# Chang-Tun-Yu/HLS-final-Visual-Odometry

Hardware: AMD Instinct MI355X
Metric: stereo frame-pairs/sec (detect+match), KITTI 1241x376; matches bit-exact (higher is better)
Workload: dtype u8; 1 GPU; KITTI 1241x376 stereo quad-match (prev/curr x L/R), default 50x50 bins; noise=0, gpu_max_hw_queues=4, streams_per_gpu=256, frames_in_hbm=8, parallelism=1x independent stream groups

## Files before the change

hls-final-visual-odometry_amd/csrc/kernels_match.hip:

```cpp
#include "vh_findmatch.h"
#include <algorithm>
#include <cstdlib>
#include <type_traits>

#ifdef VH_FLOW_STATS
__device__ unsigned long long g_flow_stats[12];
extern "C" int32_t vh_debug_flow_stats(unsigned long long *out, int32_t reset) {
  if (hipMemcpyFromSymbol(out, HIP_SYMBOL(g_flow_stats), sizeof(g_flow_stats)) != hipSuccess) return -3;
  if (reset) { unsigned long long z[12] = {0}; if (hipMemcpyToSymbol(HIP_SYMBOL(g_flow_stats), z, sizeof(z)) != hipSuccess) return -3; }
  return 0;
}
#define VH_STAT(k, n) do { if ((threadIdx.x & 63) == 0) atomicAdd(&g_flow_stats[k], (unsigned long long)(n)); } while (0)
#else
#define VH_STAT(k, n) do { } while (0)
#endif

#ifndef VH_MATCH_WAVES
#define VH_MATCH_WAVES 7
#endif
#ifndef VH_SNAKE
#define VH_SNAKE 1
#endif

namespace {

__device__ __forceinline__ int32_t wave_min(int32_t v) {
#pragma unroll
  for (int32_t d = 32; d >= 1; d >>= 1) v = min(v, __shfl_xor(v, d));
  return v;
}
__device__ __forceinline__ int32_t wave_max(int32_t v) {
#pragma unroll
  for (int32_t d = 32; d >= 1; d >>= 1) v = max(v, __shfl_xor(v, d));
  return v;
}

template <bool MAX>
__device__ __forceinline__ int32_t row16_allreduce(int32_t v) {
#define VH_ROW_STEP(CTRL)                                                                   \
  {                                                                                         \
    const int32_t t = __builtin_amdgcn_update_dpp(v, v, CTRL, 0xF, 0xF, false);             \
    v = MAX ? max(v, t) : min(v, t);                                                        \
  }
  VH_ROW_STEP(0x128)
  VH_ROW_STEP(0x124)
  VH_ROW_STEP(0x122)
  VH_ROW_STEP(0x121)
#undef VH_ROW_STEP
  return v;
}

template <class T>
__device__ __forceinline__ T ld_off(const T *base, uint32_t byte_off) { return *(const T *)((const char *)base + byte_off); }
template <class T>
__device__ __forceinline__ void st_off(T *base, uint32_t byte_off, T x) { *(T *)((char *)base + byte_off) = x; }
template <class T>
__device__ __forceinline__ T ld_uniform(const T *p) { return *(const __attribute__((address_space(4))) T *)(uintptr_t)p; }
__device__ __forceinline__ int32_t ld_uniform_i32(const int32_t *p) { return __builtin_amdgcn_readfirstlane(ld_uniform(p)); }

template <bool TESTED, class First, class Step>
__device__ __forceinline__ void walk_columns(const VhSets &s, const int32_t *__restrict__ cbs, int32_t c, int32_t UB0, int32_t UB1, int32_t VB0,
                                             int32_t VB1, int32_t ULO_MAX, int32_t UHI_MIN, int32_t VA0, int32_t VA1, First first, Step step) {
  const int32_t lane = threadIdx.x & 63;
  const bool merged = !TESTED && VB0 == 0 && VB1 == s.vbn - 1;
  const int32_t UB1w = merged ? UB0 : UB1;
  for (int32_t cb = UB0; cb <= UB1w; cb += 64) {
    const int32_t ncb = min(64, UB1w - cb + 1);
    int32_t t_p0 = 0, t_p1 = 0, t_a0 = 0, t_a1 = 0;
    if (lane < ncb) {
      const int32_t row = (c * s.ubn + cb + lane) * s.vbn;
      t_p0 = ld_off(cbs, (uint32_t)(row + VB0) * 4u);
      t_p1 = ld_off(cbs, (uint32_t)(merged ? (c * s.ubn + UB1 + 1) * s.vbn : row + VB1 + 1) * 4u);
      if (TESTED) {
        const int32_t ubx = cb + lane;
        const bool in_ = ubx * s.binsize >= ULO_MAX && ubx * s.binsize + s.binsize - 1 <= UHI_MIN;
        t_a0 = in_ ? ((VA0 <= VA1) ? cbs[row + VA0] : t_p1) : 1;
        t_a1 = in_ ? ((VA0 <= VA1) ? cbs[row + VA1 + 1] : t_p1) : 0;
      }
    }
    int32_t ci = -1, pc = -64, p1 = 0;
    const auto advance = [&]() -> bool {
      pc += 64;
      while (pc >= p1) {
        if (++ci >= ncb) return false;
        pc = __builtin_amdgcn_readlane(t_p0, ci); p1 = __builtin_amdgcn_readlane(t_p1, ci);
      }
      return true;
    };
    if (!advance()) continue;
    first(pc, p1);
    for (;;) {
      const int32_t c_pc = pc, c_p1 = p1, c_ci = ci;
      const bool more = advance();
      int32_t pa0 = 1, pa1 = 0;
      if (TESTED) { pa0 = __builtin_amdgcn_readlane(t_a0, c_ci); pa1 = __builtin_amdgcn_readlane(t_a1, c_ci); }
      step(c_pc, c_p1, pa0, pa1, more, pc, p1);
      if (!more) break;
    }
  }
}

template <bool TESTED, bool NEED_UV, class Consume>
__device__ __forceinline__ void walk_region(const VhSets &s, const int32_t *__restrict__ cbs, const uint32_t *__restrict__ cuv,
                                            const uint4 *__restrict__ cdesc, int32_t c, int32_t UB0, int32_t UB1, int32_t VB0,
                                            int32_t VB1, int32_t ULO_MAX, int32_t UHI_MIN, int32_t VA0, int32_t VA1,
                                            Consume consume) {
  const int32_t lane = threadIdx.x & 63;
  int32_t pl = 0;
  uint32_t gu = 0;
  uint4 g0, g1;
  const auto load = [&](int32_t pc, int32_t p1) __attribute__((always_inline)) {
    pl = min(pc + lane, p1 - 1);
    if (NEED_UV) gu = cuv[pl];
    g0 = cdesc[2 * (int64_t)pl]; g1 = cdesc[2 * (int64_t)pl + 1];
  };
  walk_columns<TESTED>(s, cbs, c, UB0, UB1, VB0, VB1, ULO_MAX, UHI_MIN, VA0, VA1, load,
    [&](int32_t pc, int32_t p1, int32_t pa0, int32_t pa1, bool more, int32_t npc, int32_t np1) __attribute__((always_inline)) {
      const int32_t c_pl = pl;
      const uint32_t c_gu = gu;
      const uint4 c_g0 = g0, c_g1 = g1;
      if (more) load(npc, np1);
      consume(pc, p1, pa0, pa1, c_pl, c_gu, c_g0, c_g1);
    });
}

__device__ __forceinline__ void glds16(const void *gbase, uint32_t byte_off, uint32_t lds_dst) {
  asm volatile("s_mov_b32 m0, %2\n\ts_nop 0\n\tglobal_load_lds_dwordx4 %0, %1" ::"v"(byte_off), "s"(gbase), "s"(lds_dst) : "memory");
}
__device__ __forceinline__ void glds4(const void *gbase, uint32_t byte_off, uint32_t lds_dst) {
  asm volatile("s_mov_b32 m0, %2\n\ts_nop 0\n\tglobal_load_lds_dword %0, %1" ::"v"(byte_off), "s"(gbase), "s"(lds_dst) : "memory");
}
__device__ __forceinline__ uint32_t lds_addr(const void *p) {
  return __builtin_amdgcn_readfirstlane((uint32_t)(uintptr_t)(const __attribute__((address_space(3))) void *)p);
}

template <bool TESTED, class Consume>
__device__ __forceinline__ void walk_region_lds(const VhSets &s, const int32_t *__restrict__ cbs, const uint32_t *__restrict__ cuv,
                                                const uint4 *__restrict__ cdesc, int32_t c, int32_t UB0, int32_t UB1, int32_t VB0,
                                                int32_t VB1, int32_t ULO_MAX, int32_t UHI_MIN, int32_t VA0, int32_t VA1,
                                                uint4 *wD, uint32_t *wU, Consume consume) {
  const uint32_t ldsD = lds_addr(wD), ldsU = lds_addr(wU);
  const uint32_t lane32 = (uint32_t)(threadIdx.x & 63) * 32u;
  const auto issue = [&](int32_t b, int32_t pc, int32_t p1) __attribute__((always_inline)) {
    const uint32_t off = min((uint32_t)pc * 32u + lane32, (uint32_t)(p1 - 1) * 32u);
    glds16(cdesc, off, ldsD + (uint32_t)b * 2048u); glds16(cdesc, off + 16u, ldsD + (uint32_t)b * 2048u + 1024u);
    if (TESTED) glds4(cuv, off >> 3, ldsU + (uint32_t)b * 256u);
  };
  int32_t buf = 0;
  walk_columns<TESTED>(s, cbs, c, UB0, UB1, VB0, VB1, ULO_MAX, UHI_MIN, VA0, VA1,
    [&](int32_t pc, int32_t p1) __attribute__((always_inline)) {
      asm volatile("s_waitcnt lgkmcnt(0)" ::: "memory");
      buf = 0;
      issue(0, pc, p1);
    },
    [&](int32_t pc, int32_t p1, int32_t pa0, int32_t pa1, bool more, int32_t npc, int32_t np1) __attribute__((always_inline)) {
      const int32_t c_buf = buf;
      if (more) {
        buf ^= 1;
        asm volatile("s_waitcnt lgkmcnt(0)" ::: "memory");
        issue(buf, npc, np1);
        if (TESTED) asm volatile("s_waitcnt vmcnt(3)" ::: "memory");
        else asm volatile("s_waitcnt vmcnt(2)" ::: "memory");
      } else {
        asm volatile("s_waitcnt vmcnt(0)" ::: "memory");
      }
      consume(pc, p1, pa0, pa1, (const uint4 *)(wD + c_buf * 128), (const uint32_t *)(wU + c_buf * 64));
    });
}

__device__ __forceinline__ uint64_t tested_key_uniform_query(const uint32_t (&qd)[8], us2 lo2, us2 span2, uint32_t uv2,
                                                             const uint4 &b0, const uint4 &b1, uint32_t relpos) {
  const bool out = outside_window(uv2, lo2, span2);
  const uint32_t sad = sad32(make_uint4(qd[0], qd[1], qd[2], qd[3]), make_uint4(qd[4], qd[5], qd[6], qd[7]), b0, b1, 0);
  return out ? ~0ull : (((uint64_t)sad << 32) | relpos);
}
__device__ __forceinline__ uint64_t shfl_xor_u64(uint64_t k, int32_t d) {
  const uint32_t lo = (uint32_t)__shfl_xor((int32_t)(uint32_t)k, d), hi = (uint32_t)__shfl_xor((int32_t)(uint32_t)(k >> 32), d);
  return ((uint64_t)hi << 32) | lo;
}
__device__ __forceinline__ uint64_t wave_min_u64(uint64_t k) {
#pragma unroll
  for (int32_t d = 32; d >= 1; d >>= 1) k = min(k, shfl_xor_u64(k, d));
  return k;
}

enum { KEY_HI16 = 0, KEY_W19 = 1, KEY_64 = 2 };
template <int KM> struct KeyT { typedef uint32_t type; };
template <> struct KeyT<KEY_64> { typedef uint64_t type; };
template <int KM>
__device__ __forceinline__ typename KeyT<KM>::type sad_key(const uint4 &a0, const uint4 &a1, const uint4 &b0, const uint4 &b1, uint32_t seed) {
  if (KM == KEY_HI16) return (typename KeyT<KM>::type)sad32<true>(a0, a1, b0, b1, seed);
  const uint32_t sad = sad32(a0, a1, b0, b1, 0);
  if (KM == KEY_W19) return (typename KeyT<KM>::type)((sad << 19) | seed);
  return (typename KeyT<KM>::type)(((uint64_t)sad << 32) | seed);
}
__device__ __forceinline__ int32_t key_mode_of(int32_t class_count, int32_t wide_keys) {
  if (class_count + 64 <= 0x10000 && !wide_keys) return KEY_HI16;
  return class_count <= VH_CLASS_POS_MAX && wide_keys < 2 ? KEY_W19 : KEY_64;
}

template <int Q, int P, int KM>
__device__ __forceinline__ int32_t join_phases(const typename KeyT<KM>::type (&best_key)[Q]) {
  static_assert(Q == 2 && P == 4, "the join splits the wave into two slots of two 16-lane rows");
  if (KM == KEY_64) {
    uint64_t k[Q];
#pragma unroll
    for (int32_t qi = 0; qi < Q; qi++) {
      k[qi] = (uint64_t)best_key[qi];
#pragma unroll
      for (int32_t d = 16; d < 64; d <<= 1) k[qi] = min(k[qi], shfl_xor_u64(k[qi], d));
    }
    const uint64_t kk = (threadIdx.x & 32) ? k[1] : k[0];
    return kk == ~0ull ? -1 : (int32_t)(uint32_t)kk;
  }
  const auto h = __builtin_amdgcn_permlane32_swap((uint32_t)best_key[0], (uint32_t)best_key[1], false, false);
  const uint32_t kh = min(h[0], h[1]);
  const auto r = __builtin_amdgcn_permlane16_swap(kh, kh, false, false);
  const uint32_t k = min(r[0], r[1]);
  return k == 0xFFFFFFFFu ? -1 : (int32_t)(k & (KM == KEY_HI16 ? 0xFFFFu : 0x7FFFFu));
}

#ifndef VH_REDO_G
#define VH_REDO_G 2
#endif
struct RedoGroup {
  uint32_t qd[VH_REDO_G][8];
  us2 lo2[VH_REDO_G];
  int32_t lane[VH_REDO_G], n;
  int32_t umin, umax, vmin, vmax;
};
template <int Q>
__device__ __forceinline__ bool redo_take(uint64_t &todo, const uint4 (&a0)[Q], const uint4 (&a1)[Q], const uint32_t (&uv1)[Q],
                                          int32_t radius, int32_t rv, RedoGroup &g) {
  g.n = 0; g.umin = g.vmin = 0x7FFFFFFF; g.umax = g.vmax = -1;
#pragma unroll
  for (int32_t k = 0; k < VH_REDO_G; k++) {
    if (!todo) break;
    const int32_t fl = (int32_t)__builtin_ctzll(todo), fq = fl >> 5;
    todo &= todo - 1;
    uint4 x0 = a0[0], x1 = a1[0];
    uint32_t xu = uv1[0];
#pragma unroll
    for (int32_t qi = 1; qi < Q; qi++) if (fq == qi) { x0 = a0[qi]; x1 = a1[qi]; xu = uv1[qi]; }
    g.qd[k][0] = __builtin_amdgcn_readlane(x0.x, fl); g.qd[k][1] = __builtin_amdgcn_readlane(x0.y, fl);
    g.qd[k][2] = __builtin_amdgcn_readlane(x0.z, fl); g.qd[k][3] = __builtin_amdgcn_readlane(x0.w, fl);
    g.qd[k][4] = __builtin_amdgcn_readlane(x1.x, fl); g.qd[k][5] = __builtin_amdgcn_readlane(x1.y, fl);
    g.qd[k][6] = __builtin_amdgcn_readlane(x1.z, fl); g.qd[k][7] = __builtin_amdgcn_readlane(x1.w, fl);
    const uint32_t quv1 = __builtin_amdgcn_readlane(xu, fl);
    const int32_t u1 = (int32_t)(quv1 & 0xFFFF), v1 = (int32_t)(quv1 >> 16);
    g.lo2[k] = window_lo2(quv1, radius, rv);
    g.lane[k] = fl; g.n = k + 1;
    g.umin = min(g.umin, u1); g.umax = max(g.umax, u1); g.vmin = min(g.vmin, v1); g.vmax = max(g.vmax, v1);
  }
  return g.n > 0;
}

template <int Q> struct TileOut {
  int32_t wp;
  uint4 a0[Q], a1[Q];
  uint32_t uv1[Q];
  int32_t qpos[Q];
  bool valid[Q];
};

template <int Q, int P, bool SPEC, bool FLOW>
__device__ __forceinline__ void finish_tile(const VhSets &s, const VhMatchArgs &a, int32_t pass, int32_t stream, int32_t qset, int32_t cset,
                                            int32_t c, int32_t pbase, int32_t pcnt, const TileOut<Q> &o,
                                            int32_t *__restrict__ best, int32_t *__restrict__ redo_count) {
  static_assert(Q == 2 && P == 4, "one query per lane: slot lane >> 5, on the first 16-lane row of each half (join_phases)");
  const int32_t lane = threadIdx.x & 63;
  const uint32_t *__restrict__ cuv = s.s_uv + (int64_t)cset * s.cap;
  const uint4 *__restrict__ cdesc = (const uint4 *)(s.s_desc + (int64_t)cset * s.cap * 8);
  const int32_t *__restrict__ cbs = s.bin_start + (int64_t)cset * (s.nbins + 1);
  const int32_t rv = FLOW ? a.radius : a.disp_tol;
  const us2 span2 = window_span2(a.radius, rv);
  const int32_t *__restrict__ cidx = s.s_idx + (int64_t)cset * s.cap;
  const int32_t *__restrict__ qidx = s.s_idx + (int64_t)qset * s.cap;
  int32_t *__restrict__ tbl = best + ((int64_t)stream * 4 + a.pass[pass].slot) * s.cap;
  const bool hi = lane & 32;
  const bool mine = !(lane & 16) && (hi ? o.valid[1] : o.valid[0]);
  const uint32_t uv1 = hi ? o.uv1[1] : o.uv1[0];
  const int32_t qpos = hi ? o.qpos[1] : o.qpos[0];
  int32_t res = -1;
  bool fail = false;
  if (mine && o.wp >= 0) {
    int32_t wp = o.wp;
    VH_CHECK_RANGE(s, 7, wp, 0, pcnt);
    res = pbase + wp;
    if (SPEC) fail = outside_window(ld_off(cuv, (uint32_t)res * 4u), window_lo2(uv1, a.radius, rv), span2);
  }
  if (SPEC) {
    uint64_t todo = __ballot(fail);
    if (todo) {
      const int32_t nfail = (int32_t)__popcll(todo);
      VH_STAT(FLOW ? 7 : 10, nfail);
      if (lane == 0) atomicAdd(redo_count, nfail);
      RedoGroup g;
      while (redo_take<Q>(todo, o.a0, o.a1, o.uv1, a.radius, rv, g)) {
        uint64_t kk[VH_REDO_G];
#pragma unroll
        for (int32_t k = 0; k < VH_REDO_G; k++) kk[k] = ~0ull;
        if (FLOW) {
          const VhBins b = bins_of_interest(s, VhWindow{g.umin - a.radius, g.umax + a.radius, g.vmin - rv, g.vmax + rv});
          walk_region<false, true>(s, cbs, cuv, cdesc, c, b.ub0, b.ub1, b.vb0, b.vb1, 0, 0, 0, 0,
            [&](int32_t, int32_t, int32_t, int32_t, int32_t pl, uint32_t gu, const uint4 &g0, const uint4 &g1) {
#pragma unroll
              for (int32_t k = 0; k < VH_REDO_G; k++)
                if (k < g.n) kk[k] = min(kk[k], tested_key_uniform_query(g.qd[k], g.lo2[k], span2, gu, g0, g1, (uint32_t)(pl - pbase)));
            });
        } else {
          const int32_t *__restrict__ crs = s.row_start + (int64_t)cset * (4 * s.H + 1);
          const int32_t *__restrict__ cpos = s.r_pos + (int64_t)cset * s.cap;
          const int32_t x0 = ld_uniform_i32(crs + c * s.H + max(g.vmin - rv, 0));
          const int32_t x1 = ld_uniform_i32(crs + c * s.H + min(g.vmax + rv, s.H - 1) + 1);
          for (int32_t x = x0 + lane; x < x1; x += 64) {
            int32_t cp = cpos[x];
            VH_CHECK_RANGE(s, 3, cp, pbase, pbase + pcnt);
            const uint32_t gu = cuv[cp];
            const uint4 g0 = cdesc[2 * (int64_t)cp], g1 = cdesc[2 * (int64_t)cp + 1];
#pragma unroll
            for (int32_t k = 0; k < VH_REDO_G; k++)
              if (k < g.n) kk[k] = min(kk[k], tested_key_uniform_query(g.qd[k], g.lo2[k], span2, gu, g0, g1, (uint32_t)(cp - pbase)));
          }
        }
#pragma unroll
        for (int32_t k = 0; k < VH_REDO_G; k++)
          if (k < g.n) {
            const uint64_t kf = wave_min_u64(kk[k]);
            int32_t wp = (int32_t)(uint32_t)kf;
            if (kf != ~0ull) VH_CHECK_RANGE(s, 7, wp, 0, pcnt);
            if (lane == g.lane[k]) res = kf == ~0ull ? -1 : pbase + wp;
          }
      }
    }
  }
  if (mine) st_off(tbl, (uint32_t)ld_off(qidx, (uint32_t)qpos * 4u) * 4u, res < 0 ? 0 : ld_off(cidx, (uint32_t)res * 4u));
}

template <int Q, int P, int KM, bool SPEC>
__device__ __forceinline__ void flow_tile(const VhSets &s, const VhMatchArgs &a, int32_t pass, int32_t stream,
                                          int32_t qset, int32_t cset, int32_t q0, int32_t q1, int32_t c, int32_t col0,
                                          int32_t pbase, int32_t pcnt, uint4 *wD, uint32_t *wU, TileOut<Q> &out) {
  constexpr int L = 64 / P;
  static_assert(L == 8 || L == 16, "every 16-lane row must hold the whole tile (row-wise window reduction)");
  constexpr int TRIP = 2 * P;
  const int32_t lane = threadIdx.x & 63, ph = lane / L, l = lane % L;
  const uint32_t *__restrict__ quv = s.s_uv + (int64_t)qset * s.cap;
  const uint4 *__restrict__ qdesc = (const uint4 *)(s.s_desc + (int64_t)qset * s.cap * 8);
  const uint32_t *__restrict__ cuv = s.s_uv + (int64_t)cset * s.cap;
  const uint4 *__restrict__ cdesc = (const uint4 *)(s.s_desc + (int64_t)cset * s.cap * 8);
  const int32_t *__restrict__ cbs = s.bin_start + (int64_t)cset * (s.nbins + 1);
  const int32_t rv = a.pass[pass].flow ? a.radius : a.disp_tol;

  bool (&valid)[Q] = out.valid;
  uint4 (&a0)[Q] = out.a0, (&a1)[Q] = out.a1;
  uint32_t (&uv1)[Q] = out.uv1;
  int32_t v_lo[Q];
  us2 lo2[Q];
  typedef typename KeyT<KM>::type key_t;
  const key_t KNONE = (key_t)~(key_t)0;
  key_t best_key[Q];
  int32_t umin = 0x7FFFFFFF, umax = -1, vmin = 0x7FFFFFFF, vmax = -1;
  int32_t (&qp)[Q] = out.qpos;
#pragma unroll
  for (int32_t qi = 0; qi < Q; qi++) {
    const int32_t q = q0 + L * qi + l;
    valid[qi] = q < q1;
    qp[qi] = valid[qi] ? q : q0;
  }
  {
    const int32_t *__restrict__ qbs = s.bin_start + (int64_t)qset * (s.nbins + 1);
    int32_t colb = col0, j = 0;
    int32_t csv = ld_off(qbs, (uint32_t)((c * s.ubn + min(colb + lane, s.ubn)) * s.vbn) * 4u);
    int32_t A = __builtin_amdgcn_readlane(csv, 0);
    int32_t k[Q];
#pragma unroll
    for (int32_t qi = 0; qi < Q; qi++) k[qi] = qp[qi];
    for (;;) {
      const int32_t B = __builtin_amdgcn_readlane(csv, j + 1);
      if (VH_SNAKE && ((colb + j) & 1)) {
#pragma unroll
        for (int32_t qi = 0; qi < Q; qi++) if (k[qi] >= A && k[qi] < B) qp[qi] = A + B - 1 - k[qi];
      }
      if (B >= q1 || colb + j + 1 >= s.ubn) break;
      A = B;
      if (++j == 63) { colb += 63; j = 0; csv = ld_off(qbs, (uint32_t)((c * s.ubn + min(colb + lane, s.ubn)) * s.vbn) * 4u); }
    }
  }
#pragma unroll
  for (int32_t qi = 0; qi < Q; qi++) {
    const int32_t ql = qp[qi];
    uv1[qi] = ld_off(quv, (uint32_t)ql * 4u);
    a0[qi] = ld_off(qdesc, (uint32_t)ql * 32u); a1[qi] = ld_off(qdesc, (uint32_t)ql * 32u + 16u);
    const int32_t u1 = uv1[qi] & 0xFFFF, v1 = uv1[qi] >> 16;
    v_lo[qi] = v1 - rv;
    lo2[qi] = window_lo2(uv1[qi], a.radius, rv);
    best_key[qi] = KNONE;
    umin = min(umin, u1); umax = max(umax, u1); vmin = min(vmin, v1); vmax = max(vmax, v1);
  }
  umin = __builtin_amdgcn_readfirstlane(row16_allreduce<false>(umin));
  umax = __builtin_amdgcn_readfirstlane(row16_allreduce<true>(umax));
  vmin = __builtin_amdgcn_readfirstlane(row16_allreduce<false>(vmin));
  vmax = __builtin_amdgcn_readfirstlane(row16_allreduce<true>(vmax));
  const VhBins ub = bins_of_interest(s, VhWindow{umin - a.radius, umax + a.radius, vmin - rv, vmax + rv});
  const int32_t UB0 = ub.ub0, UB1 = ub.ub1, VB0 = ub.vb0, VB1 = ub.vb1;
  const us2 span2 = window_span2(a.radius, rv);
  const int32_t ULO_MAX = umax - a.radius, UHI_MIN = umin + a.radius;
  const int32_t VLO_MAX = vmax - rv, VHI_MIN = vmin + rv;
  const int32_t VA0 = SPEC ? 0 : max(VB0, (max(VLO_MAX, 0) + s.binsize - 1) / s.binsize);
  const int32_t VA1 = SPEC ? 0 : min(VB1, (VHI_MIN + 1) / s.binsize - 1);

  auto make_key = [&](auto test, int32_t qi, uint32_t uv2, const uint4 &b0, const uint4 &b1, uint32_t seed) -> key_t {
    constexpr int TEST = decltype(test)::value;
    bool out = false;
    if (TEST == 2) {
      out = outside_window(uv2, lo2[qi], span2);
    } else if (TEST == 1) {
      out = (uint32_t)((int32_t)(uv2 >> 16) - v_lo[qi]) > (uint32_t)(2 * rv);
    }
    const key_t key = sad_key<KM>(a0[qi], a1[qi], b0, b1, seed);
    return (TEST != 0 && out) ? KNONE : key;
  };
  VH_STAT(0, 1); VH_STAT(5, q1 - q0); VH_STAT(6, UB1 - UB0 + 1);
  walk_region_lds<!SPEC>(s, cbs, cuv, cdesc, c, UB0, UB1, VB0, VB1, ULO_MAX, UHI_MIN, VA0, VA1, wD, wU,
    [&](int32_t pc, int32_t p1, int32_t pa0, int32_t pa1, const uint4 *cD, const uint32_t *cU) {
      VH_STAT(1, 1);
      const int32_t mcnt = min(64, p1 - pc);
      const int32_t jend = (mcnt + TRIP - 1) & ~(TRIP - 1);
      const uint4 *rd = cD + ph;
      const uint32_t *ru = cU + ph;
      uint32_t seedA = (uint32_t)(pc - pbase + ph), seedB = seedA + P;
      int32_t j = 0;
      auto trip = [&](auto test, int32_t o) {
        const uint4 dA0 = rd[o], dA1 = rd[o + 64], dB0 = rd[o + P], dB1 = rd[o + 64 + P];
        uint32_t uA = 0, uB = 0;
        if (decltype(test)::value != 0) { uA = ru[o]; uB = ru[o + P]; }
#pragma unroll
        for (int32_t qi = 0; qi < Q; qi++) {
          const key_t kA = make_key(test, qi, uA, dA0, dA1, seedA + (uint32_t)o), kB = make_key(test, qi, uB, dB0, dB1, seedB + (uint32_t)o);
          best_key[qi] = min(min(kA, kB), best_key[qi]);
        }
      };
      auto run = [&](auto test, int32_t jstop) {
        if (jstop > j) VH_STAT(2 + decltype(test)::value, (jstop - j) / TRIP);
        for (; j + 2 * TRIP <= jstop; j += 2 * TRIP) {
          trip(test, 0); trip(test, TRIP);
          rd += 2 * TRIP; ru += 2 * TRIP; seedA += 2 * TRIP; seedB += 2 * TRIP;
        }
        if (j < jstop) {
          trip(test, 0);
          j += TRIP; rd += TRIP; ru += TRIP; seedA += TRIP; seedB += TRIP;
        }
      };
      if (SPEC) {
        run(std::integral_constant<int, 0>{}, jend);
      } else if (pa0 <= pa1) {
        const int32_t ja = min((min(max(pa0 - pc, 0), mcnt) + TRIP - 1) & ~(TRIP - 1), jend);
        const int32_t jb = max(min(max(pa1 - pc, 0), mcnt) & ~(TRIP - 1), ja);
        run(std::integral_constant<int, 1>{}, ja);
        run(std::integral_constant<int, 0>{}, jb);
        run(std::integral_constant<int, 1>{}, jend);
      } else {
        run(std::integral_constant<int, 2>{}, jend);
      }
    });
  out.wp = join_phases<Q, P, KM>(best_key);
}

template <bool SPEC, bool FLOW, class Tile>
__device__ __forceinline__ void search_tile(const VhSets &s, const VhMatchArgs &a, int32_t pass, int32_t stream, int32_t qset, int32_t cset,
                                            int32_t c, int32_t *__restrict__ best, int32_t *__restrict__ redo_count, Tile tile) {
  const int32_t *cbs = s.bin_start + (int64_t)cset * (s.nbins + 1);
  const int32_t pbase = ld_uniform_i32(cbs + c * s.ubn * s.vbn);
  const int32_t pend = ld_uniform_i32(cbs + (c + 1) * s.ubn * s.vbn);
  const int32_t km = key_mode_of(pend - pbase, a.wide_keys);
  TileOut<VH_FLOW_Q> out;
  if (km == KEY_HI16) tile(std::integral_constant<int, KEY_HI16>{}, pbase, pend - pbase, out);
  else if (km == KEY_W19) tile(std::integral_constant<int, KEY_W19>{}, pbase, pend - pbase, out);
  else tile(std::integral_constant<int, KEY_64>{}, pbase, pend - pbase, out);
  finish_tile<VH_FLOW_Q, VH_FLOW_P, SPEC, FLOW>(s, a, pass, stream, qset, cset, c, pbase, pend - pbase, out, best, redo_count);
}

template <bool SPEC>
__device__ __forceinline__ void flow_pass(const VhSets &s, const VhMatchArgs &a, int32_t pass, int32_t stream, int32_t qset,
                                          int32_t cset, uint4 *wD, uint32_t *wU, int32_t *__restrict__ best, int32_t *__restrict__ redo_count) {
  const int32_t ntile = ld_uniform_i32(s.tile_cnt + qset);
  for (int32_t tile = __builtin_amdgcn_readfirstlane(blockIdx.x * 4 + (threadIdx.x >> 6)); tile < ntile;
       tile += gridDim.x * 4) {
    typedef int32_t i32x4 __attribute__((ext_vector_type(4)));
    const i32x4 t = ld_uniform((const i32x4 *)(s.tiles + (int64_t)qset * s.max_tiles + tile));
    const int32_t q0 = __builtin_amdgcn_readfirstlane(t.x), q1 = __builtin_amdgcn_readfirstlane(t.y);
    const int32_t c = __builtin_amdgcn_readfirstlane(t.z), col0 = __builtin_amdgcn_readfirstlane(t.w);
    search_tile<SPEC, true>(s, a, pass, stream, qset, cset, c, best, redo_count,
      [&](auto km, int32_t pbase, int32_t pcnt, TileOut<VH_FLOW_Q> &out) __attribute__((always_inline)) {
        flow_tile<VH_FLOW_Q, VH_FLOW_P, decltype(km)::value, SPEC>(s, a, pass, stream, qset, cset, q0, q1, c, col0, pbase, pcnt, wD, wU, out);
      });
  }
}

template <int Q, int P, int KM, bool SPEC>
__device__ __forceinline__ void rows_tile(const VhSets &s, const VhMatchArgs &a, int32_t pass, int32_t stream, int32_t qset,
                                          int32_t cset, int32_t q0, int32_t q1, int32_t c, int32_t pbase, int32_t pcnt, uint4 *wD,
                                          uint32_t *wU, uint32_t *wV, TileOut<Q> &out) {
  constexpr int L = 64 / P;
  static_assert(L == 8 || L == 16, "every 16-lane row must hold the whole tile");
  constexpr int TRIP = 2 * P;
  const int32_t lane = threadIdx.x & 63, ph = lane / L, l = lane % L;
  const int32_t nrow = 4 * s.H;
  const int32_t *__restrict__ crs = s.row_start + (int64_t)cset * (nrow + 1);
  const int32_t *__restrict__ qpos = s.r_pos + (int64_t)qset * s.cap;
  const uint32_t *__restrict__ quv = s.s_uv + (int64_t)qset * s.cap;
  const uint4 *__restrict__ qdesc = (const uint4 *)(s.s_desc + (int64_t)qset * s.cap * 8);
  const int32_t *__restrict__ cpos = s.r_pos + (int64_t)cset * s.cap;
  const uint32_t *__restrict__ cuv = s.s_uv + (int64_t)cset * s.cap;
  const uint4 *__restrict__ cdesc = (const uint4 *)(s.s_desc + (int64_t)cset * s.cap * 8);

  bool (&valid)[Q] = out.valid;
  uint4 (&a0)[Q] = out.a0, (&a1)[Q] = out.a1;
  uint32_t (&uv1)[Q] = out.uv1;
  int32_t (&qp)[Q] = out.qpos;
  typedef typename KeyT<KM>::type key_t;
  key_t best_key[Q];
  us2 lo2[Q];
  const us2 span2 = window_span2(a.radius, a.disp_tol);
  int32_t vmin = 0x7FFFFFFF, vmax = -1;
#pragma unroll
  for (int32_t qi = 0; qi < Q; qi++) {
    const int32_t q = q0 + L * qi + l;
    valid[qi] = q < q1;
    qp[qi] = ld_off(qpos, (uint32_t)(valid[qi] ? q : q0) * 4u);
    VH_CHECK_RANGE(s, 1, qp[qi], 0, s.cap);
    uv1[qi] = ld_off(quv, (uint32_t)qp[qi] * 4u);
    a0[qi] = ld_off(qdesc, (uint32_t)qp[qi] * 32u); a1[qi] = ld_off(qdesc, (uint32_t)qp[qi] * 32u + 16u);
    const int32_t v1 = uv1[qi] >> 16;
    lo2[qi] = window_lo2(uv1[qi], a.radius, a.disp_tol);
    best_key[qi] = (key_t)~(key_t)0;
    vmin = min(vmin, v1); vmax = max(vmax, v1);
  }
  vmin = __builtin_amdgcn_readfirstlane(row16_allreduce<false>(vmin));
  vmax = __builtin_amdgcn_readfirstlane(row16_allreduce<true>(vmax));
  VH_STAT(8, 1); VH_STAT(11, q1 - q0);
  const int32_t VLO = max(vmin - a.disp_tol, 0), VHI = min(vmax + a.disp_tol, s.H - 1);
  const int32_t r0 = ld_uniform_i32(crs + c * s.H + VLO);
  const int32_t r1 = ld_uniform_i32(crs + c * s.H + VHI + 1);
  for (int32_t rc = r0; rc < r1; rc += 64) {
    const int32_t mcnt = min(64, r1 - rc);
    int32_t cp = ld_off(cpos, (uint32_t)min(rc + lane, r1 - 1) * 4u);
    VH_CHECK_RANGE(s, 2, cp, pbase, pbase + pcnt);
    const uint4 g0 = ld_off(cdesc, (uint32_t)cp * 32u), g1 = ld_off(cdesc, (uint32_t)cp * 32u + 16u);
    uint32_t gu = 0;
    if (!SPEC) gu = ld_off(cuv, (uint32_t)cp * 4u);
    asm volatile("s_waitcnt lgkmcnt(0)" ::: "memory");
    wD[lane] = g0; wD[64 + lane] = g1; wU[lane] = (uint32_t)(cp - pbase);
    if (!SPEC) wV[lane] = gu;
    asm volatile("s_waitcnt lgkmcnt(0)" ::: "memory");
    const int32_t jend = (mcnt + TRIP - 1) & ~(TRIP - 1);
    VH_STAT(9, jend / TRIP);
    const uint4 *rd = wD + ph;
    const uint32_t *ru = wU + ph, *rv = wV + ph;
    for (int32_t j = 0; j < jend; j += TRIP) {
      const uint4 dA0 = rd[0], dA1 = rd[64], dB0 = rd[P], dB1 = rd[64 + P];
      const uint32_t sA = ru[0], sB = ru[P];
      uint32_t uA = 0, uB = 0;
      if (!SPEC) { uA = rv[0]; uB = rv[P]; }
#pragma unroll
      for (int32_t qi = 0; qi < Q; qi++) {
        key_t kA = sad_key<KM>(a0[qi], a1[qi], dA0, dA1, sA), kB = sad_key<KM>(a0[qi], a1[qi], dB0, dB1, sB);
        if (!SPEC) {
          kA = outside_window(uA, lo2[qi], span2) ? (key_t)~(key_t)0 : kA;
          kB = outside_window(uB, lo2[qi], span2) ? (key_t)~(key_t)0 : kB;
        }
        best_key[qi] = min(min(kA, kB), best_key[qi]);
      }
      rd += TRIP; ru += TRIP; rv += TRIP;
    }
  }
  out.wp = join_phases<Q, P, KM>(best_key);
}

template <bool SPEC>
__device__ __forceinline__ void rows_pass(const VhSets &s, const VhMatchArgs &a, int32_t pass, int32_t stream, int32_t qset,
                                          int32_t cset, uint4 *wD, uint32_t *wU, uint32_t *wV, int32_t *__restrict__ best, int32_t *__restrict__ redo_count) {
  const int32_t nrow = 4 * s.H;
  const int32_t *__restrict__ qrs = s.row_start + (int64_t)qset * (nrow + 1);
  int32_t cls_q0[5];
#pragma unroll
  for (int32_t c = 0; c <= 4; c++) cls_q0[c] = ld_uniform_i32(qrs + c * s.H);
  constexpr int T = VH_TILE_Q;
  for (int32_t tile = __builtin_amdgcn_readfirstlane(blockIdx.x * 4 + (threadIdx.x >> 6));; tile += gridDim.x * 4) {
    int32_t c = -1, q0 = 0, q1 = 0, t = tile;
#pragma unroll
    for (int32_t k = 0; k < 4; k++) {
      const int32_t nt = (cls_q0[k + 1] - cls_q0[k] + T - 1) / T;
      if (c < 0 && t < nt) { c = k; q0 = cls_q0[k] + T * t; q1 = min(cls_q0[k + 1], q0 + T); }
      if (c < 0) t -= nt;
    }
    if (c < 0) break;
    search_tile<SPEC, false>(s, a, pass, stream, qset, cset, c, best, redo_count,
      [&](auto km, int32_t pbase, int32_t pcnt, TileOut<VH_FLOW_Q> &out) __attribute__((always_inline)) {
        rows_tile<VH_FLOW_Q, VH_FLOW_P, decltype(km)::value, SPEC>(s, a, pass, stream, qset, cset, q0, q1, c, pbase, pcnt, wD, wU, wV, out);
      });
  }
}

template <bool SPEC>
__global__ void __launch_bounds__(256) __attribute__((amdgpu_waves_per_eu(VH_MATCH_WAVES, 8)))
match_kernel(VhSets s, VhMatchArgs a, int32_t *__restrict__ best, int32_t *__restrict__ redo) {
  __shared__ uint4 sDesc[4 * 256];
  __shared__ uint32_t sAux[4 * 128];
  __shared__ uint32_t sAux2[SPEC ? 1 : 4 * 64];
  const int32_t pass = blockIdx.y, stream = blockIdx.z;
  if (a.prior && pass == 1) return;
#ifdef VH_EXP_SKIP
  if (VH_EXP_SKIP & (a.pass[pass].flow ? 2 : 1)) return;
#endif
  const int32_t qset = vh_row_set(a, stream, a.pass[pass].qset);
  const int32_t cset = vh_row_set(a, stream, a.pass[pass].cset);
  uint4 *wD = sDesc + (threadIdx.x >> 6) * 256;
  uint32_t *wU = sAux + (threadIdx.x >> 6) * 128;
  uint32_t *wV = sAux2 + (SPEC ? 0 : (threadIdx.x >> 6) * 64);
  int32_t *redo_count = redo + stream;
  if (a.pass[pass].flow) flow_pass<SPEC>(s, a, pass, stream, qset, cset, wD, wU, best, redo_count);
  else rows_pass<SPEC>(s, a, pass, stream, qset, cset, wD, wU, wV, best, redo_count);
}

}

void vh_launch_match(const VhSets &s, const VhMatchArgs &a, int32_t *best, int32_t *redo, int32_t speculative, int32_t grid_x,
                     int32_t lds_bytes, hipStream_t st) {
  if (!a.npass) return;
  VhMatchArgs m = a;
  static const int wide = [] { const char *e = getenv("VH_FLOW_WIDE_KEYS"); return e ? atoi(e) : 0; }();
  m.wide_keys = wide;
  static const int wgs = [] { const char *e = getenv("VH_FLOW_WGS"); return e ? atoi(e) : 0; }();
  static const int pad_env = [] { const char *e = getenv("VH_FLOW_LDS_PAD"); return e ? atoi(e) : -1; }();
  const int32_t gx = wgs > 0 ? wgs : (grid_x > 0 ? (grid_x | 1) : (((s.max_tiles + 3) / 4) | 1));
  dim3 grid(gx, m.npass, a.rows);
  static const size_t static_lds[2] = {
      [] { hipFuncAttributes at{}; return hipFuncGetAttributes(&at, (const void *)match_kernel<false>) == hipSuccess ? at.sharedSizeBytes : (size_t)0; }(),
      [] { hipFuncAttributes at{}; return hipFuncGetAttributes(&at, (const void *)match_kernel<true>) == hipSuccess ? at.sharedSizeBytes : (size_t)0; }()};
  const size_t have = static_lds[speculative ? 1 : 0];
  const int32_t pad = pad_env >= 0 ? pad_env : (wgs > 0 || grid_x <= 0 || lds_bytes <= 0 || have == 0 || (size_t)lds_bytes <= have ? 0 : (int32_t)((size_t)lds_bytes - have));
  if (speculative) hipLaunchKernelGGL(match_kernel<true>, grid, dim3(256), pad, st, s, m, best, redo);
  else hipLaunchKernelGGL(match_kernel<false>, grid, dim3(256), pad, st, s, m, best, redo);
}
```

Measured before the change: 115,900 pairs/s.

## Double-buffer candidate descriptor loads in rows_tile via async global-to-LDS DMA

Replaces the synchronous load-then-store of candidate descriptors into LDS with direct global-to-LDS loads (glds16/glds4) into two alternating buffers. Candidate positions are prefetched two chunks ahead, so the next chunk's fetch overlaps the SAD scan of the current chunk. The goal is to hide global memory latency and drop the register round-trip through VGPRs. In exchange it doubles the wV LDS buffer for the non-speculative path and depends on hand-counted vmcnt waits, which are fragile if the number of outstanding loads changes.

```diff
diff --git a/hls-final-visual-odometry_amd/csrc/kernels_match.hip b/hls-final-visual-odometry_amd/csrc/kernels_match.hip
--- a/hls-final-visual-odometry_amd/csrc/kernels_match.hip
+++ b/hls-final-visual-odometry_amd/csrc/kernels_match.hip
@@ -543,36 +543,60 @@
   const int32_t VLO = max(vmin - a.disp_tol, 0), VHI = min(vmax + a.disp_tol, s.H - 1);
   const int32_t r0 = ld_uniform_i32(crs + c * s.H + VLO);
   const int32_t r1 = ld_uniform_i32(crs + c * s.H + VHI + 1);
-  for (int32_t rc = r0; rc < r1; rc += 64) {
-    const int32_t mcnt = min(64, r1 - rc);
-    int32_t cp = ld_off(cpos, (uint32_t)min(rc + lane, r1 - 1) * 4u);
-    VH_CHECK_RANGE(s, 2, cp, pbase, pbase + pcnt);
-    const uint4 g0 = ld_off(cdesc, (uint32_t)cp * 32u), g1 = ld_off(cdesc, (uint32_t)cp * 32u + 16u);
-    uint32_t gu = 0;
-    if (!SPEC) gu = ld_off(cuv, (uint32_t)cp * 4u);
+  if (r0 < r1) {
+    const uint32_t ldsD = lds_addr(wD), ldsV = lds_addr(wV);
+    const auto load_cp = [&](int32_t rc) __attribute__((always_inline)) {
+      int32_t cp = ld_off(cpos, (uint32_t)min(rc + lane, r1 - 1) * 4u);
+      VH_CHECK_RANGE(s, 2, cp, pbase, pbase + pcnt);
+      return cp;
+    };
+    const auto issue = [&](int32_t b, int32_t cp) __attribute__((always_inline)) {
+      glds16(cdesc, (uint32_t)cp * 32u, ldsD + (uint32_t)b * 2048u); glds16(cdesc, (uint32_t)cp * 32u + 16u, ldsD + (uint32_t)b * 2048u + 1024u);
+      if (!SPEC) glds4(cuv, (uint32_t)cp * 4u, ldsV + (uint32_t)b * 256u);
+      wU[b * 64 + lane] = (uint32_t)(cp - pbase);
+    };
+    constexpr int NDMA = SPEC ? 2 : 3;
+    int32_t cpn = load_cp(r0), cpn2 = cpn;
+    if (r0 + 64 < r1) cpn2 = load_cp(r0 + 64);
     asm volatile("s_waitcnt lgkmcnt(0)" ::: "memory");
-    wD[lane] = g0; wD[64 + lane] = g1; wU[lane] = (uint32_t)(cp - pbase);
-    if (!SPEC) wV[lane] = gu;
-    asm volatile("s_waitcnt lgkmcnt(0)" ::: "memory");
-    const int32_t jend = (mcnt + TRIP - 1) & ~(TRIP - 1);
-    VH_STAT(9, jend / TRIP);
-    const uint4 *rd = wD + ph;
-    const uint32_t *ru = wU + ph, *rv = wV + ph;
-    for (int32_t j = 0; j < jend; j += TRIP) {
-      const uint4 dA0 = rd[0], dA1 = rd[64], dB0 = rd[P], dB1 = rd[64 + P];
-      const uint32_t sA = ru[0], sB = ru[P];
-      uint32_t uA = 0, uB = 0;
-      if (!SPEC) { uA = rv[0]; uB = rv[P]; }
-#pragma unroll
-      for (int32_t qi = 0; qi < Q; qi++) {
-        key_t kA = sad_key<KM>(a0[qi], a1[qi], dA0, dA1, sA), kB = sad_key<KM>(a0[qi], a1[qi], dB0, dB1, sB);
-        if (!SPEC) {
-          kA = outside_window(uA, lo2[qi], span2) ? (key_t)~(key_t)0 : kA;
-          kB = outside_window(uB, lo2[qi], span2) ? (key_t)~(key_t)0 : kB;
+    issue(0, cpn);
+    cpn = cpn2;
+    for (int32_t rc = r0, b = 0;; rc += 64, b ^= 1) {
+      const bool more = rc + 64 < r1;
+      if (more) {
+        asm volatile("s_waitcnt lgkmcnt(0)" ::: "memory");
+        issue(b ^ 1, cpn);
+        if (rc + 128 < r1) {
+          cpn = load_cp(rc + 128);
+          asm volatile("s_waitcnt vmcnt(%0)" ::"n"(NDMA + 1) : "memory");
+        } else {
+          asm volatile("s_waitcnt vmcnt(%0)" ::"n"(NDMA) : "memory");
         }
-        best_key[qi] = min(min(kA, kB), best_key[qi]);
-      }
-      rd += TRIP; ru += TRIP; rv += TRIP;
+      } else {
+        asm volatile("s_waitcnt vmcnt(0)" ::: "memory");
+      }
+      const int32_t mcnt = min(64, r1 - rc);
+      const int32_t jend = (mcnt + TRIP - 1) & ~(TRIP - 1);
+      VH_STAT(9, jend / TRIP);
+      const uint4 *rd = wD + b * 128 + ph;
+      const uint32_t *ru = wU + b * 64 + ph, *rv = wV + b * 64 + ph;
+      for (int32_t j = 0; j < jend; j += TRIP) {
+        const uint4 dA0 = rd[0], dA1 = rd[64], dB0 = rd[P], dB1 = rd[64 + P];
+        const uint32_t sA = ru[0], sB = ru[P];
+        uint32_t uA = 0, uB = 0;
+        if (!SPEC) { uA = rv[0]; uB = rv[P]; }
+#pragma unroll
+        for (int32_t qi = 0; qi < Q; qi++) {
+          key_t kA = sad_key<KM>(a0[qi], a1[qi], dA0, dA1, sA), kB = sad_key<KM>(a0[qi], a1[qi], dB0, dB1, sB);
+          if (!SPEC) {
+            kA = outside_window(uA, lo2[qi], span2) ? (key_t)~(key_t)0 : kA;
+            kB = outside_window(uB, lo2[qi], span2) ? (key_t)~(key_t)0 : kB;
+          }
+          best_key[qi] = min(min(kA, kB), best_key[qi]);
+        }
+        rd += TRIP; ru += TRIP; rv += TRIP;
+      }
+      if (!more) break;
     }
   }
   out.wp = join_phases<Q, P, KM>(best_key);
@@ -608,7 +632,7 @@
 match_kernel(VhSets s, VhMatchArgs a, int32_t *__restrict__ best, int32_t *__restrict__ redo) {
   __shared__ uint4 sDesc[4 * 256];
   __shared__ uint32_t sAux[4 * 128];
-  __shared__ uint32_t sAux2[SPEC ? 1 : 4 * 64];
+  __shared__ uint32_t sAux2[SPEC ? 1 : 4 * 128];
   const int32_t pass = blockIdx.y, stream = blockIdx.z;
   if (a.prior && pass == 1) return;
 #ifdef VH_EXP_SKIP
@@ -618,7 +642,7 @@
   const int32_t cset = vh_row_set(a, stream, a.pass[pass].cset);
   uint4 *wD = sDesc + (threadIdx.x >> 6) * 256;
   uint32_t *wU = sAux + (threadIdx.x >> 6) * 128;
-  uint32_t *wV = sAux2 + (SPEC ? 0 : (threadIdx.x >> 6) * 64);
+  uint32_t *wV = sAux2 + (SPEC ? 0 : (threadIdx.x >> 6) * 128);
   int32_t *redo_count = redo + stream;
   if (a.pass[pass].flow) flow_pass<SPEC>(s, a, pass, stream, qset, cset, wD, wU, best, redo_count);
   else rows_pass<SPEC>(s, a, pass, stream, qset, cset, wD, wU, wV, best, redo_count);
```

Result: faster. 117,400 pairs/s, median of 6 (+1.3%).
